# twke18/SPML

Measured on AMD Instinct MI355X. Metric: images/sec (513x513) + k-means iters/sec, higher is better.
Workload: dtype f32

## Files before the change

### include/spml_hip.h

```cpp
#ifndef SPML_HIP_H_
#define SPML_HIP_H_

#include <stddef.h>
#include <stdint.h>

#ifdef __cplusplus
extern "C" {
#endif

typedef enum spml_status {
  SPML_OK = 0,
  SPML_ERR_INVALID_ARG = -1,
  SPML_ERR_UNSUPPORTED = -2,
  SPML_ERR_WORKSPACE = -3,
  SPML_ERR_LAUNCH = -4
} spml_status;

const char* spml_status_string(int status);

#define SPML_ABI_VERSION 8
int spml_abi_version(void);

int spml_set_deterministic(int on);
int spml_get_deterministic(void);
// ... 337 lines not shown

int spml_bn_bwd_hl8_f32(const float* dy, const float* y, const unsigned char* relu_mask,
                        const float* x, int64_t R, int C, const float* mean,
                        const float* invstd, const float* gamma, const float* cmax,
                        const float* cmin, float* d_gamma, float* d_beta, float* dx,
                        void* dx_hl8, float* dx_bound, float* d_residual, void* ws,
                        size_t ws_bytes, void* stream);

int spml_bn_bwd_hl8_chunks_f32(const float* dy, const unsigned char* relu_mask, const float* x,
                               const float* chunk_stats, int chunks, int chunk_rows, int64_t R,
                               int C, const float* mean, const float* invstd, const float* gamma,
                               const float* cmax, const float* cmin, float* d_gamma,
                               float* d_beta, float* max_dz, float* dx, void* dx_hl8,
                               float* dx_bound, float* d_residual, void* stream);

int spml_bn_act_bwd_reduce_ext_chunks_f32(const float* chunk_stats, int chunks, int chunk_rows,
                                          int64_t R, int C, const float* invstd, float* sum_dz,
                                          float* sum_dz_xhat, float* max_dz, void* stream);

int spml_conv_hl8_pyramid_f32(const void* a, const float* a_bound, const void* b,
                              const float* b_bound, const float* bias, const float* addend,
                              float* out,
                              int n_img, int H, int W, int K, int N, int groups,
                              const int* dilations, void* stream);
int spml_hl8_weight_transposed_into_f32(const float* w, int Cout, int taps, int Cin,
                                        const float* bound, void* out, int taps_total,
                                        int tap_offset, void* stream);
int spml_absmax_bound_f32(const float* x, int64_t n, float* bound, int zero_first,
                          void* stream);

int spml_hl8_weight_set_f32(const float* const* w, const int* cout, const int* cin,
                            const int* taps, int n, float* bounds, void* const* fwd,
                            void* const* transposed, void* stream);

int spml_bn_finalize_ranks_f32(const float* stats, int world, int C, float eps,
                               float momentum, float* running_mean, float* running_var,
                               float* mean, float* invstd, float* total_count, void* stream);

int spml_conv_hl8_affine_f32(const void* a, const float* a_bound, const void* b,
                             const float* b_bound, const float* bias, const float* addend,
                             int relu, float* out, float* out_bound, int n_img, int H,
                             int W, int K, int N, int taps, int dilation, void* stream);

int spml_upsample_ce_supported(int C);
size_t spml_upsample_ce_workspace_bytes(int N, int H, int W);
int spml_upsample_ce_fwd_f32(const float* logits, const int64_t* labels, int N, int C, int h,
                             int w, int H, int W, int64_t ignore_index, float* lse,
                             float* result, void* ws, size_t ws_bytes, void* stream);
int spml_upsample_ce_bwd_f32(const float* logits, const int64_t* labels, const float* lse,
                             int N, int C, int h, int w, int H, int W, int64_t ignore_index,
                             const float* scale, float* d_logits, void* stream);
const char* spml_upsample_ce_bwd_path_name(int N, int C, int h, int w, int H, int W);


int spml_unit_hl8_from_nchw_f32(const float* x, int n, int C, int h, int w, void* out,
                                void* stream);

int spml_class_head_supported(int Ch, int ncls);

int spml_class_head_accumulate_f32(const float* hidden, int Ch, int h, int w,
                                   const float* weight, const float* bias, int ncls,
                                   float* canvas, int Hp, int Wp, int sh, int sw,
                                   void* stream);

int spml_argmax_channels_i64(const float* canvas, int ncls, int Hp, int Wp, int h, int w,
                             int64_t* out, void* stream);
// ... 103 lines not shown
```

### spml_amd/_ffi.py

```python
import ctypes
import os
import threading
from ctypes import c_char_p, c_double, c_float, c_int, c_int64, c_size_t, c_void_p

import torch

_HERE = os.path.dirname(os.path.abspath(__file__))
LIB_PATH = os.environ.get('SPML_HIP_LIB') or os.path.join(_HERE, 'lib', 'libspml_hip.so')

_lib = None
_lock = threading.Lock()

_P = c_void_p
_SIGNATURES = {
    'spml_status_string': (c_char_p, [c_int]),
    'spml_abi_version': (c_int, []),
    'spml_normalize_concat_loc_f32': (c_int, [_P, c_int, c_int, c_int, c_int, _P, _P, _P, _P, _P]),
    'spml_normalize_concat_loc_bwd_f32': (c_int, [_P, c_int, c_int, c_int, c_int, _P, _P, _P, _P, _P, _P]),
    'spml_normalize_concat_local_f32': (c_int, [_P, c_int, c_int, c_int, c_int, _P, c_int, _P, _P, _P, _P]),
    'spml_normalize_concat_local_nhwc_supported': (c_int, [c_int, c_int]),
    'spml_normalize_concat_local_nhwc_f32': (c_int, [_P, c_int, c_int, c_int, c_int, _P, c_int, _P, _P, _P, _P]),
    'spml_normalize_concat_local_nhwc_bwd_f32': (c_int, [_P, c_int, c_int, c_int, c_int, _P, c_int, _P, _P, _P,
                                                         _P, _P]),
    'spml_normalize_concat_local_bwd_f32': (c_int, [_P, c_int, c_int, c_int, c_int, _P, c_int, _P, _P, _P,
# ... 59 lines not shown
                                                   c_int, c_int, c_int, _P, _P, _P]),
    'spml_bn_bwd_hl8_chunks_f32': (c_int, [_P, _P, _P, _P, c_int, c_int, c_int64, c_int, _P, _P, _P, _P, _P, _P, _P, _P,
                                           _P, _P, _P, _P, _P]),
    'spml_bn_act_bwd_reduce_ext_chunks_f32': (c_int, [_P, c_int, c_int, c_int64, c_int, _P, _P, _P, _P, _P]),
    'spml_conv_wgrad_hl8_supported': (c_int, [c_int, c_int, c_int]),
    'spml_conv_wgrad_workspace_bytes': (c_size_t, [c_int, c_int, c_int, c_int, c_int, c_int]),
    'spml_conv_wgrad_hl8_f32': (c_int, [_P, _P, _P, _P, _P, c_int, c_int, c_int, c_int, c_int, c_int, c_int, _P,
                                        c_size_t, _P]),
    'spml_conv_wgrad_pyramid_hl8_supported': (c_int, [c_int, c_int, c_int]),
    'spml_conv_tap_gather_f32': (c_int, [_P, _P, _P, c_int, c_int, c_int, c_int, c_int, _P, _P]),
    'spml_conv_wgrad_pyramid_workspace_bytes': (c_size_t, [c_int, c_int, c_int, c_int, c_int, c_int]),
    'spml_conv_wgrad_pyramid_hl8_f32': (c_int, [_P, _P, _P, _P, _P, c_int, c_int, c_int, c_int, c_int, c_int, _P, _P,
                                                c_size_t, _P]),
    'spml_conv_hl8_path_name': (c_char_p, [c_int, c_int, c_int, c_int, c_int, c_int, c_int, c_int]),
    'spml_conv_wgrad_path_name': (c_char_p, [c_int, c_int, c_int, c_int, c_int, c_int, c_int]),
    'spml_conv_wgrad_splits': (c_int, [c_int, c_int, c_int, c_int, c_int, c_int, c_int]),
    'spml_bn_stats_ext_f32': (c_int, [_P, c_int64, c_int, _P, _P, _P, _P, _P, c_size_t, _P]),
    'spml_bn_stats_ext_chunks_f32': (c_int, [_P, c_int, c_int, c_int64, c_int, _P, _P, _P, _P, _P]),
    'spml_bn_finalize_f32': (c_int, [_P, _P, c_int, c_double, c_float, c_float, _P, _P, _P, _P]),
    'spml_bn_act_apply_hl8_f32': (c_int, [_P, _P, _P, c_int64, c_int, _P, _P, _P, _P, _P, _P, c_int, _P, _P, _P, _P,
                                          _P]),
    'spml_bn_act_bwd_reduce_ext_f32': (c_int, [_P, _P, _P, _P, c_int64, c_int, _P, _P, _P, _P, _P, _P, c_size_t, _P]),
    'spml_bn_act_bwd_apply_hl8_f32': (c_int, [_P, _P, _P, _P, c_int64, c_int, _P, _P, _P, _P, _P, _P, _P, _P,
                                              c_double, _P, _P, _P, _P, _P, _P]),
    'spml_bn_fwd_hl8_f32': (c_int, [_P, _P, _P, c_int64, c_int, _P, _P, _P, _P, c_float, c_float, c_int, _P, _P, _P, _P,
                                    _P, _P, _P, _P, _P, c_size_t, _P]),
    'spml_bn_bwd_hl8_f32': (c_int, [_P, _P, _P, _P, c_int64, c_int, _P, _P, _P, _P, _P, _P, _P, _P, _P, _P, _P, _P,
                                    c_size_t, _P]),
    'spml_conv_hl8_pyramid_f32': (c_int, [_P, _P, _P, _P, _P, _P, _P, c_int, c_int, c_int, c_int, c_int, c_int, _P,
                                          _P]),
    'spml_hl8_weight_transposed_into_f32': (c_int, [_P, c_int, c_int, c_int, _P, _P, c_int, c_int, _P]),
    'spml_absmax_bound_f32': (c_int, [_P, c_int64, _P, c_int, _P]),
    'spml_hl8_weight_set_f32': (c_int, [_P, _P, _P, _P, c_int, _P, _P, _P, _P]),
    'spml_bn_finalize_ranks_f32': (c_int, [_P, c_int, c_int, c_float, c_float, _P, _P, _P, _P, _P, _P]),
    'spml_conv_hl8_affine_f32': (c_int, [_P, _P, _P, _P, _P, _P, c_int, _P, _P, c_int, c_int, c_int, c_int, c_int,
                                         c_int, c_int, _P]),
    'spml_upsample_ce_supported': (c_int, [c_int]),
    'spml_upsample_ce_workspace_bytes': (c_size_t, [c_int, c_int, c_int]),
    'spml_upsample_ce_fwd_f32': (c_int, [_P, _P, c_int, c_int, c_int, c_int, c_int, c_int, c_int64, _P, _P, _P,
                                         c_size_t, _P]),
    'spml_upsample_ce_bwd_f32': (c_int, [_P, _P, _P, c_int, c_int, c_int, c_int, c_int, c_int, c_int64, _P, _P, _P]),
    'spml_upsample_ce_bwd_path_name': (c_char_p, [c_int, c_int, c_int, c_int, c_int, c_int]),
    'spml_bn_stats_f32': (c_int, [_P, c_int64, c_int, _P, _P, _P, c_size_t, _P]),
    'spml_bn_act_apply_f32': (c_int, [_P, _P, c_int64, c_int, _P, _P, _P, _P, c_int, _P, _P]),
    'spml_bn_act_bwd_reduce_f32': (c_int, [_P, _P, _P, c_int64, c_int, _P, _P, _P, _P, _P, c_size_t, _P]),
    'spml_bn_act_bwd_apply_f32': (c_int, [_P, _P, _P, c_int64, c_int, _P, _P, _P, _P, _P, c_double, _P, _P, _P,
                                          _P]),
    'spml_clock_probe': (c_int, [_P, c_int, _P]),
    'spml_maxpool3x3s2_nhwc_f32': (c_int, [_P, c_int, c_int, c_int, c_int, _P, _P]),
    'spml_window_accumulate_f32': (c_int, [_P, c_int, c_int, c_int, _P, _P, c_int, c_int, c_int, c_int,
                                           _P]),
    'spml_unit_hl8_from_nchw_f32': (c_int, [_P, c_int, c_int, c_int, c_int, _P, _P]),
    'spml_class_head_supported': (c_int, [c_int, c_int]),
    'spml_class_head_accumulate_f32': (c_int, [_P, c_int, c_int, c_int, _P, _P, c_int, _P, c_int, c_int, c_int, c_int,
                                               _P]),
    'spml_argmax_channels_i64': (c_int, [_P, c_int, c_int, c_int, c_int, c_int, _P, _P]),
    'spml_iou_counts_i64': (c_int, [_P, _P, c_int64, c_int, _P, _P]),
    'spml_resample_unit_f32': (c_int, [_P, c_int, c_int, c_int, c_int64, c_int64, c_int64, c_int, c_int, c_int, c_int,
                                       c_int, _P, c_int, c_int, _P]),
    'spml_resample_classes_accumulate_f32': (c_int, [_P, c_int, c_int, c_int, c_int64, c_int64, c_int64, c_int, c_int,
                                                     c_int, c_int, c_int, c_int, _P, _P]),
    'spml_cam_finalize_f32': (c_int, [_P, c_int, c_int64, c_int, c_int, _P, c_int, c_float, _P, _P]),
    'spml_upsample_argmax_i64': (c_int, [_P, c_int, c_int, c_int, c_int, c_int, _P, _P]),
    'spml_view_probs_accumulate_f32': (c_int, [_P, c_int, c_int, c_int, _P, _P, c_int, c_int, c_int, c_int, c_int, _P,
                                               _P]),
    'spml_view_votes_workspace_bytes': (c_size_t, [c_int, c_int]),
# ... 1152 lines not shown
                                  versions=tuple(wt._version for wt in weights), operand=operand)
  z = conv_hl8(x, operand, n_img, h, w, 1)
  bias = None
  if any(bb is not None for bb in biases):
    bias = sum(bb.detach() for bb in biases if bb is not None).contiguous()
  out = torch.empty((n_img, cout, h, w), dtype=torch.float32, device=dev, memory_format=torch.channels_last)
  dil = (ctypes.c_int * groups)(*[int(d) for d in dilations])
  check(lib().spml_conv_tap_gather_f32(_ptr_any(z), _dp(bias), _ptr_any(out), n_img, h, w, cout, groups,
                                       ctypes.cast(dil, c_void_p), stream_ptr()), 'spml_conv_tap_gather_f32')
  return out


def hl8_weight_set(weights):
  import ctypes
  n = len(weights)
  dev = weights[0].device
  wl = [wt.detach().contiguous(memory_format=torch.channels_last) for wt in weights]
  bounds = torch.empty((4,), dtype=torch.float32, device=dev)
  shapes = [(wt.shape[0], wt.shape[1], wt.shape[2] * wt.shape[3]) for wt in wl]
  fwd = [torch.empty((co * ci * t * 4,), dtype=torch.uint8, device=dev) for co, ci, t in shapes]
  tr = [torch.empty((co * ci * t * 4,), dtype=torch.uint8, device=dev) for co, ci, t in shapes]
  pv, iv = ctypes.c_void_p * n, ctypes.c_int * n
  check(lib().spml_hl8_weight_set_f32(
      pv(*[wt.data_ptr() for wt in wl]), iv(*[sh[0] for sh in shapes]), iv(*[sh[1] for sh in shapes]),
      iv(*[sh[2] for sh in shapes]), n, _dp(bounds), pv(*[t.data_ptr() for t in fwd]),
      pv(*[t.data_ptr() for t in tr]), stream_ptr()), 'spml_hl8_weight_set_f32')
  out = []
  for i, (co, ci, t) in enumerate(shapes):
    b = bounds[i:i + 1]
    out.append((Hl8(fwd[i], b, co, t * ci), Hl8(tr[i], b, ci, t * co)))
  return out


def conv_hl8_affine(a, b, bias, n_img, h, w, taps, dilation=1, addend=None, relu=True, want_hl8=True):
  k, n = a.channels, b.rows
  if a.rows != n_img * h * w or b.channels != taps * k:
    raise SpmlHipError('conv_hl8_affine: operand shapes do not match')
  dev = a.data.device
  out = torch.empty((n_img, n, h, w), dtype=torch.float32, device=dev, memory_format=torch.channels_last)
  bound = _f32(1, dev) if want_hl8 else None
  check(lib().spml_conv_hl8_affine_f32(ptr(a.data), _dp(a.bound), ptr(b.data), _dp(b.bound), ptr(bias, torch.float32),
                                       _ptr_any(addend, True), int(bool(relu)), _ptr_any(out), _dp(bound), n_img, h, w,
                                       k, n, taps, dilation, stream_ptr()), 'spml_conv_hl8_affine_f32')
  return out, (hl8_from_f32(out, bound=bound) if want_hl8 else None)


def upsample_ce_supported(c):
  return bool(lib().spml_upsample_ce_supported(int(c)))


def upsample_ce_bwd_path_name(n, c, h, w, hh, ww):
  return lib().spml_upsample_ce_bwd_path_name(int(n), int(c), int(h), int(w), int(hh), int(ww)).decode()


def upsample_ce_fwd(logits_nhwc, labels, ignore_index):
  n, h, w, c = logits_nhwc.shape
  hh, ww = labels.shape[-2:]
  lse = torch.empty((n, hh, ww), dtype=torch.float32, device=logits_nhwc.device)
  result = torch.empty((3,), dtype=torch.float32, device=logits_nhwc.device)
  ws = workspace(lib().spml_upsample_ce_workspace_bytes(n, hh, ww), logits_nhwc.device)
  check(lib().spml_upsample_ce_fwd_f32(ptr(logits_nhwc, torch.float32), ptr(labels, torch.int64), n, c, h, w, hh, ww,
                                       int(ignore_index), ptr(lse), ptr(result), ptr(ws), ws.numel(), stream_ptr()),
        'spml_upsample_ce_fwd_f32')
  return result, lse


# ... 281 lines not shown
```

### spml_amd/csrc/conv.hip

```cpp
#include "common.hpp"

#include <math.h>
#include <stdlib.h>

#ifndef SPML_CONV_EXP
#define SPML_CONV_EXP 0
#endif

namespace spml {
namespace {

constexpr int BSTAT_BATCH = 8;

typedef const __attribute__((address_space(1))) void* gptr_t;
typedef __attribute__((address_space(3))) void* lptr_t;

__device__ uint4 g_zero_page[16];

__device__ __forceinline__ float pow2_scale(float bound) {
  if (!(bound > 0.f) || bound > 1e38f) return 1.f;
  int e;
  (void)frexpf(bound, &e);
  e = 14 - e;
  e = e < -100 ? -100 : (e > 100 ? 100 : e);
// ... 90 lines not shown
  for (int o = 32; o > 0; o >>= 1) m = fmaxf(m, __shfl_xor(m, o, kWave));
  if ((threadIdx.x & 63) == 0) sm[threadIdx.x >> 6] = m;
  __syncthreads();
  if (threadIdx.x == 0)
    atomicMax(reinterpret_cast<unsigned*>(ws.bound + wi), __float_as_uint(fmaxf(fmaxf(sm[0], sm[1]), fmaxf(sm[2], sm[3]))));
}

__global__ __launch_bounds__(256) void weightset_convert(const WeightSet ws) {
  const int64_t total = ws.start[ws.n];
  for (int64_t i = (int64_t)blockIdx.x * 256 + threadIdx.x; i < total; i += (int64_t)gridDim.x * 256) {
    int wi = 0;
    while (wi + 1 < ws.n && i >= ws.start[wi + 1]) ++wi;
    const int64_t u = i - ws.start[wi];
    const int cout = ws.cout[wi], cin = ws.cin[wi], taps = ws.taps[wi];
    const float s = pow2_scale(ws.bound[wi]);
    const float4v v0 = reinterpret_cast<const float4v*>(ws.w[wi])[2 * u];
    const float4v v1 = reinterpret_cast<const float4v*>(ws.w[wi])[2 * u + 1];
    const float v[8] = {v0[0], v0[1], v0[2], v0[3], v1[0], v1[1], v1[2], v1[3]};
    union { half8 h; uint4 q; _Float16 e[8]; } hh, ll;
    split_unscaled(v, s, hh.h, ll.h);
    ws.fwd[wi][2 * u] = hh.q;
    ws.fwd[wi][2 * u + 1] = ll.q;
    const int c8 = cin >> 3;
    const int ci0 = (int)(u % c8) * 8;
    const int64_t rest = u / c8;
    const int tap = (int)(rest % taps), co = (int)(rest / taps);
    const int tapo = taps - 1 - tap;
    _Float16* th = reinterpret_cast<_Float16*>(ws.tr[wi]);
#pragma unroll
    for (int e = 0; e < 8; ++e) {
      const size_t tu = ((size_t)(ci0 + e) * taps + tapo) * (cout >> 3) + (co >> 3);
      th[(2 * tu) * 8 + (co & 7)] = hh.e[e];
      th[(2 * tu + 1) * 8 + (co & 7)] = ll.e[e];
    }
  }
}

struct ConvArgs {
  const uint4* a;
  const uint4* b;
  const float* a_bound;
  const float* b_bound;
  const float* addend;
  const unsigned char* addend_mask;
  const float* bias;
  int relu;
  float* out_bound;
  float* out;
  int64_t R;
  int H, W, K, N, taps, dil;
  int n_col_tiles, n_tiles;
  int dils[4];
  int tap_groups;
  float* stats;
  float* stats_zero;
  const float* bstat_x;
  const unsigned char* bstat_mask;
  const float* bstat_mean;
  float* bstats;
};

template <int RB, int kStages, int WGS, int RG, bool CHUNK = false, int NC = 4, bool BSTAT = false, bool BADD = false>
__global__ __launch_bounds__(64 * NC * RG, WGS) void conv_gemm(const ConvArgs a) {
  static_assert(!BSTAT || (RG == 1 && NC == 4), "backward statistics: a wave owns its 64 columns over the whole tile");
  static_assert(!BADD || (BSTAT && !CHUNK), "the addend form exists for the un-chunked backward statistics only");
  constexpr int kABlocks = 2 * RB * RG;
// ... 874 lines not shown
  hipLaunchKernelGGL(hl8_convert_wt, dim3(grid), dim3(256), 0, (hipStream_t)stream, w, Cout, taps, Cin, bound,
                     static_cast<uint4*>(out), taps_total, tap_offset);
  return launch_status();
}

extern "C" int spml_hl8_weight_set_f32(const float* const* w, const int* cout, const int* cin, const int* taps,
                                       int n, float* bounds, void* const* fwd, void* const* transposed,
                                       void* stream) {
  if (!w || !cout || !cin || !taps || !bounds || !fwd || !transposed || n < 1 || n > 4) return SPML_ERR_INVALID_ARG;
  WeightSet ws{};
  ws.n = n;
  ws.bound = bounds;
  int64_t acc = 0, largest = 0;
  for (int i = 0; i < n; ++i) {
    if (!w[i] || !fwd[i] || !transposed[i] || cout[i] <= 0 || cin[i] <= 0 || (taps[i] != 1 && taps[i] != 9))
      return SPML_ERR_INVALID_ARG;
    if ((cout[i] & 7) || (cin[i] & 7) || !al16(w[i]) || !al16(fwd[i]) || !al16(transposed[i])) return SPML_ERR_UNSUPPORTED;
    ws.w[i] = w[i];
    ws.fwd[i] = static_cast<uint4*>(fwd[i]);
    ws.tr[i] = static_cast<uint4*>(transposed[i]);
    ws.cout[i] = cout[i]; ws.cin[i] = cin[i]; ws.taps[i] = taps[i];
    ws.start[i] = acc;
    const int64_t units = (int64_t)cout[i] * cin[i] * taps[i] / 8;
    acc += units;
    largest = std::max(largest, units);
  }
  for (int i = n; i <= 4; ++i) ws.start[i] = acc;
  hipStream_t s = (hipStream_t)stream;
  if (hipMemsetAsync(bounds, 0, 4 * sizeof(float), s) != hipSuccess) return SPML_ERR_LAUNCH;
  const int gx = (int)std::min<int64_t>(256, (largest * 2 + 255) / 256);
  hipLaunchKernelGGL(weightset_absmax, dim3(gx, n), dim3(256), 0, s, ws);
  const int grid = (int)std::min<int64_t>(4096, (acc + 255) / 256);
  hipLaunchKernelGGL(weightset_convert, dim3(grid), dim3(256), 0, s, ws);
  return launch_status();
}

extern "C" int spml_absmax_bound_f32(const float* x, int64_t n, float* bound, int zero_first, void* stream) {
  if (!x || !bound || n <= 0) return SPML_ERR_INVALID_ARG;
  if (!al16(x)) return SPML_ERR_UNSUPPORTED;
  hipStream_t s = (hipStream_t)stream;
  if (zero_first && hipMemsetAsync(bound, 0, sizeof(float), s) != hipSuccess) return SPML_ERR_LAUNCH;
  const int grid = (int)std::min<int64_t>(2048, (n / 4 + 255) / 256 + 1);
  hipLaunchKernelGGL(absmax_bound, dim3(grid), dim3(256), 0, s, x, n, reinterpret_cast<unsigned*>(bound));
  return launch_status();
}

extern "C" int spml_conv_hl8_supported(int K, int N, int taps) {
  return (taps == 1 || taps == 9) && K > 0 && (K & 15) == 0 && N > 0 && (N & 63) == 0;
}

extern "C" int spml_conv_hl8_f32(const void* a, const float* a_bound, const void* b, const float* b_bound,
                                 const float* addend, const unsigned char* addend_mask, float* out, int n_img,
                                 int H, int W, int K, int N, int taps, int dilation, void* stream) {
  if (!a || !b || !out || n_img <= 0 || H <= 0 || W <= 0 || dilation < 1) return SPML_ERR_INVALID_ARG;
  if (!spml_conv_hl8_supported(K, N, taps) || !al16(a) || !al16(b) || !al16(out) || (addend && !al16(addend)))
    return SPML_ERR_UNSUPPORTED;
  ConvArgs c{};
  c.a = static_cast<const uint4*>(a);
  c.b = static_cast<const uint4*>(b);
  c.a_bound = a_bound;
  c.b_bound = b_bound;
  c.addend = addend;
  c.addend_mask = addend ? addend_mask : nullptr;
  c.out = out;
  c.R = (int64_t)n_img * H * W;
  c.H = H; c.W = W; c.K = K; c.N = N; c.taps = taps; c.dil = dilation;
// ... 320 lines not shown
```

### spml_amd/mc_bottleneck.py

```python
import os

import torch
import torch.distributed as dist

from spml_amd import _ffi
from spml_amd._cache import BoundedCache


def _group_of(bn):
  if isinstance(bn, torch.nn.SyncBatchNorm) and dist.is_available() and dist.is_initialized():
    return bn.process_group if bn.process_group is not None else dist.group.WORLD
  return None


def available(block, x, allow_forward_only=True):
  if os.environ.get('SPML_NO_MC_CONV') == '1' or not (x.is_cuda and x.dtype == torch.float32 and x.dim() == 4):
    return False
  if not block.training or block.stride != 1 or not x.is_contiguous(memory_format=torch.channels_last):
    return False
  convs = [block.conv1, block.conv2, block.conv3] + ([block.downsample[0]] if block.downsample is not None else [])
  if os.environ.get('SPML_MC_NARROW_UNITS') == '0' and any(
      (c.in_channels & 255) or (c.out_channels & 255) for c in convs):
    return False
  bns = [block.bn1, block.bn2, block.bn3] + ([block.downsample[1]] if block.downsample is not None else [])
# ... 176 lines not shown
  side.wait_stream(main)
  with torch.cuda.stream(side):
    dw = _ffi.conv_wgrad_hl8(dy, x, n, h, w, taps, dil)
  dy.data.record_stream(side)
  dy.bound.record_stream(side)
  dw.record_stream(main)
  return dw


def handover_mode():
  return 0 if os.environ.get('SPML_BN3_HANDOVER') == '0' else 1


class _Handover(object):
  taken = 0

  def __init__(self):
    self.bn3 = None
    self.dx = self.stats = self.version = None

  def put(self, dx, stats):
    self.dx, self.stats, self.version = dx, stats, dx._version

  def take(self, d_out):
    dx, stats, version = self.dx, self.stats, self.version
    self.dx = self.stats = self.version = None
    if dx is None or d_out._version != version or d_out.data_ptr() != dx.data_ptr() or d_out.shape != dx.shape or \
        d_out.stride() != dx.stride() or d_out.dtype != dx.dtype:
      return None
    _Handover.taken += 1
    return stats


class _Unit(torch.autograd.Function):

  @staticmethod
  def forward(ctx, block, x, xh_data, xh_bound, w1, g1, b1, w2, g2, b2, w3, g3, b3, wd, gd, bd, hand_out=None,
              hand_in=None, *p_bn3):
    n, cin, h, w = x.shape
    rows = n * h * w
    dil = block.conv2.dilation[0]
    width, cout = w1.shape[0], w3.shape[0]
    xh = _ffi.Hl8(xh_data, xh_bound, rows, cin) if xh_data is not None else _ffi.hl8_from_f32(x)
    wset = _ffi.hl8_weight_set([w1, w2, w3] + ([wd] if wd is not None else []))
    (w1f, w1t), (w2f, w2t), (w3f, w3t) = wset[:3]
    conv = _ffi.conv_hl8_stats
    a1, s1 = conv(xh, w1f, n, h, w, 1)
    counters = []
    n1 = _Bn(block.bn1, a1, rows, width, chunk_stats=s1, counters=counters)
    a2, s2 = conv(n1.yh, w2f, n, h, w, 9, dil)
    n2 = _Bn(block.bn2, a2, rows, width, chunk_stats=s2, counters=counters)
    a3, s3 = conv(n2.yh, w3f, n, h, w, 1)
    nd = ad = wdt = None
    ex3 = None
    if wd is not None:
      wdf, wdt = wset[3]
      ad, sd = conv(xh, wdf, n, h, w, 1)
      ex3, exd = sync_pair(block.bn3, a3, s3, block.downsample[1], ad, sd, rows, cout)
      nd = _Bn(block.downsample[1], ad, rows, cout, relu=False, want_f32=True, want_hl8=False, chunk_stats=sd,
               counters=counters, gathered=exd)
      residual, res_bound = nd.y, nd.bound
    else:
      residual, res_bound = x, xh.bound
    n3 = _Bn(block.bn3, a3, rows, cout, residual=residual, residual_bound=res_bound, want_f32=True, chunk_stats=s3,
             counters=counters, gathered=ex3)
    bump_counters(counters)
    ctx.block, ctx.geom = block, (n, cin, h, w, dil, width, cout)
    ctx.bn_meta = [(m.count, m.group, m.world) for m in (n1, n2, n3)] + \
        ([(nd.count, nd.group, nd.world)] if nd is not None else [])
    tensors = [xh.data, xh.bound, a1, n1.yh.data, n1.yh.bound, a2, n2.yh.data, n2.yh.bound, a3, n3.mask,
               n1.mask, n2.mask,
               w1t.data, w1t.bound, w2t.data, w2t.bound, w3t.data, w3t.bound, g1, g2, g3]
    tensors += list(n1.saved) + list(n2.saved) + list(n3.saved)
    if nd is not None:
      tensors += [ad, wdt.data, wdt.bound, gd] + list(nd.saved)
    ctx.hand_in = ctx.hand_out = None
    if hand_in is not None and len(p_bn3) == 3 and p_bn3[0] is not None and n3.world == 1 and \
# ... 54 lines not shown
    dw1 = _wgrad(side, da1, xh, n, h, w, 1)
    dx = None
    if p_bn3 is not None and need_x and handover_mode():
      last = lambda dy, wt, **kw: _ffi.conv_hl8_bwd_stats(dy, wt, n, h, w, 1, 1, p_bn3[0], p_bn3[1], p_bn3[2], **kw)
    else:
      last = lambda dy, wt, **kw: (_ffi.conv_hl8(dy, wt, n, h, w, 1, **kw), None)
    cx = None
    if has_ds:
      ad, wdt_d, wdt_b, gd = t[33:37]
      sd = t[37:41]
      if not pair:
        _, dad, _, dgd, dbd = _bn_backward(dres, ad, rows, cout, gd, sd, m[3][0], m[3][1], m[3][2], None)
      dwd = _wgrad(side, dad, xh, n, h, w, 1)
      if need_x:
        dx = _ffi.conv_hl8(da1, w1t, n, h, w, 1)
        dx, cx = last(dad, H(wdt_d, wdt_b, cin, cout), addend=dx)
    elif need_x:
      dx, cx = last(da1, w1t, addend=d_out, addend_mask=m3)
    if cx is not None:
      ctx.hand_in.put(dx, cx)
    if side is not None:
      torch.cuda.current_stream().wait_stream(side)
    return (None, dx, None, None, dw1, dg1, db1, dw2, dg2, db2, dw3, dg3, db3, dwd, dgd, dbd) + (None,) * 5


class _ConvBnAct(torch.autograd.Function):

  @staticmethod
  def forward(ctx, conv, bn, x, weight, gamma, beta):
    n, cin, h, w = x.shape
    rows, cout = n * h * w, weight.shape[0]
    taps, dil = weight.shape[2] * weight.shape[3], conv.dilation[0]
    xh = getattr(x, '_spml_hl8', None) or _ffi.hl8_from_f32(x)
    (wf, wt), = _ffi.hl8_weight_set([weight])
    a, st = _ffi.conv_hl8_stats(xh, wf, n, h, w, taps, dil)
    nb = _Bn(bn, a, rows, cout, relu=True, want_f32=True, want_hl8=False, chunk_stats=st)
    ctx.geom = (n, cin, h, w, taps, dil, cout)
    ctx.bn_meta = (nb.count, nb.group, nb.world)
    ctx.save_for_backward(xh.data, xh.bound, a, nb.mask, wt.data, wt.bound, gamma, *nb.saved)
    return nb.y

  @staticmethod
  def backward(ctx, dy):
    n, cin, h, w, taps, dil, cout = ctx.geom
    rows = n * h * w
    xh_d, xh_b, a, mask, wt_d, wt_b, gamma = ctx.saved_tensors[:7]
    saved = ctx.saved_tensors[7:11]
    if not dy.is_contiguous(memory_format=torch.channels_last):
      dy = dy.contiguous(memory_format=torch.channels_last)
    count, group, world = ctx.bn_meta
    _, da, _, dg, db = _bn_backward(dy, a, rows, cout, gamma, saved, count, group, world, mask)
    side = _side_stream(dy.device)
    dw = _wgrad(side, da, _ffi.Hl8(xh_d, xh_b, rows, cin), n, h, w, taps, dil)
    dx = None
    if ctx.needs_input_grad[2]:
      dx = _ffi.conv_hl8(da, _ffi.Hl8(wt_d, wt_b, cin, taps * cout), n, h, w, taps, dil)
    if side is not None:
      torch.cuda.current_stream().wait_stream(side)
    return None, None, dx, dw, dg, db


def conv_bn_act_available(conv, bn, x):
  if os.environ.get('SPML_NO_MC_CONV') == '1' or not (x.is_cuda and x.dtype == torch.float32 and x.dim() == 4):
    return False
  if not (bn.training and torch.is_grad_enabled() and x.is_contiguous(memory_format=torch.channels_last)):
    return False
  k = conv.kernel_size
# ... 29 lines not shown
```

### spml_amd/nn/optimizer.py

```python
import torch
from torch.optim.optimizer import Optimizer, required


class SGD(Optimizer):

  def __init__(self, params, lr=required, momentum=0, dampening=0, weight_decay=0,
               nesterov=False):
    if nesterov and (momentum <= 0 or dampening != 0):
      raise ValueError('Nesterov momentum requires a momentum and zero dampening')
    assert dampening == 0, 'not implemented'
    defaults = dict(lr=lr, momentum=momentum, dampening=dampening,
                    weight_decay=weight_decay, nesterov=nesterov)
    super().__init__(params, defaults)

  @torch.no_grad()
  def step(self, lr, closure=None):
    loss = None
    if closure is not None:
      with torch.enable_grad():
        loss = closure()
    for group in self.param_groups:
      params = [p for p in group['params'] if p.grad is not None]
      if not params:
        continue
      grads = [p.grad for p in params]
      wd, mom, scale = group['weight_decay'], group['momentum'], group['lr'] * lr
      if wd != 0:
        grads = torch._foreach_add(grads, params, alpha=wd)
      if mom != 0:
        bufs = []
        for p in params:
          st = self.state[p]
          if 'momentum_buffer' not in st:
            st['momentum_buffer'] = torch.zeros_like(p)
          bufs.append(st['momentum_buffer'])
        torch._foreach_mul_(bufs, mom)
        torch._foreach_add_(bufs, grads, alpha=scale)
        if group['nesterov']:
          upd = torch._foreach_add(grads, bufs, alpha=mom)
        else:
          upd = bufs
        torch._foreach_sub_(params, upd)
      else:
        torch._foreach_sub_(params, grads)
    return loss
```

### spml_amd/train.py

```python
import os

import torch
import torch.distributed as dist

import spml_amd.models.utils as model_utils
import spml_amd.utils.general.train as train_utils
from spml_amd import parallel
from spml_amd.models.embeddings.resnet_deeplab import resnet_50_deeplab, resnet_101_deeplab
from spml_amd.models.embeddings.resnet_pspnet import resnet_50_pspnet, resnet_101_pspnet
from spml_amd.models.predictions import segsort as segsort_plain
from spml_amd.models.predictions import segsort_softmax
from spml_amd.nn.optimizer import SGD

LOSS_KEYS = ('sem_ann_loss', 'sem_occ_loss', 'img_sim_loss', 'feat_aff_loss')


def build_models(config, softmax_head=True, recipe='voc'):
  backbone = config.network.backbone_types
  if recipe == 'densepose':
    import spml_amd.models.embeddings.resnet_pspnet_densepose as dp_emb
    import spml_amd.models.predictions.segsort_softmax_densepose as dp_pred
    makers = {'panoptic_pspnet_101': dp_emb.resnet_101_pspnet,
              'panoptic_pspnet_50': dp_emb.resnet_50_pspnet}
    if backbone not in makers:
# ... 12 lines not shown
  else:
    raise ValueError('Not support ' + str(backbone))
  if config.network.prediction_types == 'segsort':
    prediction_model = (segsort_softmax if softmax_head else segsort_plain).segsort(config)
  else:
    raise ValueError('Not support ' + str(config.network.prediction_types))
  return embedding_model, prediction_model


class Trainer:

  def __init__(self, config, device, softmax_head=True, freeze_unused=True,
               channels_last=False, recipe='voc', models=None):
    self.config = config
    self.device = torch.device(device)
    self.distributed = parallel.is_distributed()
    self.world = dist.get_world_size() if self.distributed else 1
    emb, pred = models if models is not None else build_models(config, softmax_head, recipe)
    if freeze_unused:
      for name in ('conv1', 'res2'):
        for p in getattr(emb.resnet_backbone, name).parameters():
          p.requires_grad_(False)
    emb, pred = emb.to(self.device), pred.to(self.device)
    if channels_last:
      emb = emb.to(memory_format=torch.channels_last)
      pred = pred.to(memory_format=torch.channels_last)
    if config.network.use_syncbn and self.distributed:
      emb = torch.nn.SyncBatchNorm.convert_sync_batchnorm(emb)
      pred = torch.nn.SyncBatchNorm.convert_sync_batchnorm(pred)
    self.embedding_model, self.prediction_model = emb, pred
    self.optimizer = SGD(emb.get_params_lr() + pred.get_params_lr(), lr=1,
                         momentum=config.train.momentum,
                         weight_decay=config.train.weight_decay)
    self.emb_fwd, self.pred_fwd = emb, pred
    if self.distributed:
      ids = [self.device.index] if self.device.type == 'cuda' else None
      ddp = dict(device_ids=ids, broadcast_buffers=not config.network.use_syncbn,
                 gradient_as_bucket_view=True, bucket_cap_mb=64)
      self.emb_fwd = torch.nn.parallel.DistributedDataParallel(emb, **ddp)
      if any(p.requires_grad for p in pred.parameters()):
        self.pred_fwd = torch.nn.parallel.DistributedDataParallel(pred, **ddp)
    self.memory_banks = {}
    self.curr_iter = config.train.begin_iteration
    if self.device.type == 'cuda':
      from spml_amd import _ffi
      if _ffi.deterministic():
        from spml_amd.nn.conv import make_deterministic
        make_deterministic(self.embedding_model)
        make_deterministic(self.prediction_model)
      if _ffi.deterministic() and os.environ.get('SPML_DETERMINISTIC_FRAMEWORK') == '1':
        torch.backends.cudnn.deterministic = True
        torch.backends.cudnn.benchmark = False

  def lr(self, it):
    t = self.config.train
    if t.lr_policy == 'step':
      return train_utils.lr_step(t.base_lr, it, t.decay_iterations, t.warmup_iteration)
    return train_utils.lr_poly(t.base_lr, it, t.max_iteration, t.warmup_iteration)

  def forward_losses(self, datas, targets):
    targets = dict(targets)
    emb = self.emb_fwd(datas, targets)
    protos = model_utils.local_prototypes(
        emb['cluster_embedding'], emb['cluster_embedding_with_loc'], emb['cluster_index'],
        emb['cluster_batch_index'], emb['cluster_semantic_label'], emb['cluster_instance_label'])
    (targets['prototype'], targets['prototype_with_loc'], targets['prototype_semantic_label'],
# ... 52 lines not shown
        'prediction_model': self.prediction_model.state_dict(),
        'optimizer': self.optimizer.state_dict(),
        'memory_banks': self.memory_banks,
        'iteration': self.curr_iter,
    }



class ClassifierTrainer:

  def __init__(self, config, device, channels_last=False, models=None):
    from spml_amd.models.predictions.softmax_classifier import softmax_classifier
    self.config = config
    self.device = torch.device(device)
    self.distributed = parallel.is_distributed()
    if models is not None:
      emb, pred = models
    else:
      if config.network.prediction_types != 'softmax_classifier':
        raise ValueError('Not support ' + str(config.network.prediction_types))
      makers = {'panoptic_pspnet_101': resnet_101_pspnet, 'panoptic_deeplab_101': resnet_101_deeplab}
      if config.network.backbone_types not in makers:
        raise ValueError('Not support ' + str(config.network.backbone_types))
      emb, pred = makers[config.network.backbone_types](config), softmax_classifier(config)
    emb, pred = emb.to(self.device), pred.to(self.device)
    if channels_last:
      emb = emb.to(memory_format=torch.channels_last)
      pred = pred.to(memory_format=torch.channels_last)
    if config.network.use_syncbn and self.distributed:
      pred = torch.nn.SyncBatchNorm.convert_sync_batchnorm(pred)
    self.embedding_model, self.prediction_model = emb, pred
    self.optimizer = SGD(emb.get_params_lr() + pred.get_params_lr(), lr=1,
                         momentum=config.train.momentum, weight_decay=config.train.weight_decay)
    if self.device.type == 'cuda':
      from spml_amd import _ffi
      if _ffi.deterministic():
        from spml_amd.nn.conv import make_deterministic
        make_deterministic(pred)
        make_deterministic(emb)
    self.pred_fwd = pred
    if self.distributed:
      ids = [self.device.index] if self.device.type == 'cuda' else None
      self.pred_fwd = torch.nn.parallel.DistributedDataParallel(
          pred, device_ids=ids, broadcast_buffers=not config.network.use_syncbn)
    self.curr_iter = config.train.begin_iteration

  lr = Trainer.lr

  def load_pretrained(self, path_or_state):
    state = path_or_state
    if isinstance(state, (str, bytes)) or hasattr(state, '__fspath__'):
      state = torch.load(state, map_location=self.device, weights_only=True)
    if 'embedding_model' not in state:
      raise ValueError('Pre-trained model is required.')
    self.embedding_model.load_state_dict(state['embedding_model'], resume=True)

  def step(self, datas, targets):
    self.embedding_model.eval()
    self.prediction_model.train()
    with torch.no_grad():
      embeddings = self.embedding_model.generate_embeddings(datas, targets)
    outputs = self.pred_fwd({'embedding': embeddings['embedding']}, targets)
    loss = outputs['sem_ann_loss']
    lr = self.lr(self.curr_iter)
    self.optimizer.zero_grad()
    loss.backward()
# ... 66 lines not shown
```

Before: 147.6.

## Batch per-step weight splitting into one table launch and fuse SGD updates

Adds a multi-tensor SGD kernel that updates every parameter, with weight decay and momentum, in a few launches instead of per-tensor PyTorch ops. It also adds a forward pre-hook that, at the start of each model forward, converts all conv weights seen in the previous forward to the split half format in one batched absmax/convert pass. Convolution units then look those results up instead of launching per-block conversions. The aim is to cut kernel launch and Python overhead. The cost is extra hook bookkeeping, and the weight table only takes effect after the first forward has recorded which weights were requested.

```diff
diff --git a/include/spml_hip.h b/include/spml_hip.h
--- a/include/spml_hip.h
+++ b/include/spml_hip.h
@@ -393,6 +393,14 @@
 int spml_hl8_weight_set_f32(const float* const* w, const int* cout, const int* cin,
                             const int* taps, int n, float* bounds, void* const* fwd,
                             void* const* transposed, void* stream);
+
+int spml_hl8_weight_table_f32(const float* const* w, const int* cout, const int* cin,
+                              const int* taps, int n, float* bounds, void* const* fwd,
+                              void* const* transposed, void* stream);
+
+int spml_sgd_step_f32(void* const* p, const void* const* grad, void* const* buf,
+                      const int64_t* numel, const float* scale, const float* weight_decay,
+                      const float* momentum, int n, void* stream);
 
 int spml_bn_finalize_ranks_f32(const float* stats, int world, int C, float eps,
                                float momentum, float* running_mean, float* running_var,
diff --git a/spml_amd/_ffi.py b/spml_amd/_ffi.py
--- a/spml_amd/_ffi.py
+++ b/spml_amd/_ffi.py
@@ -115,6 +115,8 @@
     'spml_hl8_weight_transposed_into_f32': (c_int, [_P, c_int, c_int, c_int, _P, _P, c_int, c_int, _P]),
     'spml_absmax_bound_f32': (c_int, [_P, c_int64, _P, c_int, _P]),
     'spml_hl8_weight_set_f32': (c_int, [_P, _P, _P, _P, c_int, _P, _P, _P, _P]),
+    'spml_hl8_weight_table_f32': (c_int, [_P, _P, _P, _P, c_int, _P, _P, _P, _P]),
+    'spml_sgd_step_f32': (c_int, [_P, _P, _P, _P, _P, _P, _P, c_int, _P]),
     'spml_bn_finalize_ranks_f32': (c_int, [_P, c_int, c_int, c_float, c_float, _P, _P, _P, _P, _P, _P]),
     'spml_conv_hl8_affine_f32': (c_int, [_P, _P, _P, _P, _P, _P, c_int, _P, _P, c_int, c_int, c_int, c_int, c_int,
                                          c_int, c_int, _P]),
@@ -1333,6 +1335,44 @@
   return out
 
 
+def hl8_weight_table(weights):
+  import ctypes
+  n = len(weights)
+  dev = weights[0].device
+  wl = [wt.detach().contiguous(memory_format=torch.channels_last) for wt in weights]
+  shapes = [(wt.shape[0], wt.shape[1], wt.shape[2] * wt.shape[3]) for wt in wl]
+  sizes = [co * ci * t * 4 for co, ci, t in shapes]
+  offs = [0]
+  for sz in sizes:
+    offs.append(offs[-1] + (sz + 255) // 256 * 256)
+  bounds = torch.empty((n,), dtype=torch.float32, device=dev)
+  fwd = torch.empty((offs[-1],), dtype=torch.uint8, device=dev)
+  tr = torch.empty((offs[-1],), dtype=torch.uint8, device=dev)
+  pv, iv = ctypes.c_void_p * n, ctypes.c_int * n
+  f0, t0 = fwd.data_ptr(), tr.data_ptr()
+  check(lib().spml_hl8_weight_table_f32(
+      pv(*[wt.data_ptr() for wt in wl]), iv(*[sh[0] for sh in shapes]), iv(*[sh[1] for sh in shapes]),
+      iv(*[sh[2] for sh in shapes]), n, _dp(bounds), pv(*[f0 + o for o in offs[:-1]]),
+      pv(*[t0 + o for o in offs[:-1]]), stream_ptr()), 'spml_hl8_weight_table_f32')
+  out = []
+  for i, (co, ci, t) in enumerate(shapes):
+    b = bounds[i:i + 1]
+    out.append((Hl8(fwd[offs[i]:offs[i] + sizes[i]], b, co, t * ci), Hl8(tr[offs[i]:offs[i] + sizes[i]], b, ci, t * co)))
+  return out
+
+
+def sgd_step(params, grads, bufs, scales, weight_decays, momenta):
+  import ctypes
+  n = len(params)
+  if n == 0:
+    return
+  pv, fv = ctypes.c_void_p * n, ctypes.c_float * n
+  check(lib().spml_sgd_step_f32(
+      pv(*[t.data_ptr() for t in params]), pv(*[t.data_ptr() for t in grads]),
+      pv(*[None if t is None else t.data_ptr() for t in bufs]), (ctypes.c_int64 * n)(*[t.numel() for t in params]),
+      fv(*scales), fv(*weight_decays), fv(*momenta), n, stream_ptr()), 'spml_sgd_step_f32')
+
+
 def conv_hl8_affine(a, b, bias, n_img, h, w, taps, dilation=1, addend=None, relu=True, want_hl8=True):
   k, n = a.channels, b.rows
   if a.rows != n_img * h * w or b.channels != taps * k:
diff --git a/spml_amd/csrc/conv.hip b/spml_amd/csrc/conv.hip
--- a/spml_amd/csrc/conv.hip
+++ b/spml_amd/csrc/conv.hip
@@ -146,6 +146,101 @@
       const size_t tu = ((size_t)(ci0 + e) * taps + tapo) * (cout >> 3) + (co >> 3);
       th[(2 * tu) * 8 + (co & 7)] = hh.e[e];
       th[(2 * tu + 1) * 8 + (co & 7)] = ll.e[e];
+    }
+  }
+}
+
+struct WeightRow {
+  const float* w;
+  uint4* fwd;
+  uint4* tr;
+  float* bound;
+  int32_t cout, cin, taps;
+};
+constexpr int WT_ROWS = 72;
+struct WeightBatch {
+  WeightRow row[WT_ROWS];
+  int start[WT_ROWS + 1];
+  int n;
+};
+static_assert(sizeof(WeightBatch) <= 4000, "the batch must fit the kernel argument segment");
+
+constexpr int WT_CO = 64, WT_CI = 32;
+constexpr int WT_LD = WT_CO + 8;
+
+__device__ __forceinline__ int weighttable_row(const WeightBatch& b) {
+  int wi = 0, hi = b.n;
+  while (hi - wi > 1) {
+    const int mid = (wi + hi) >> 1;
+    if ((int)blockIdx.x >= b.start[mid]) wi = mid; else hi = mid;
+  }
+  return wi;
+}
+
+__global__ __launch_bounds__(256) void weighttable_absmax(const WeightBatch b) {
+  __shared__ float sm[4];
+  const int wi = weighttable_row(b);
+  const WeightRow& r = b.row[wi];
+  const int q = (int)blockIdx.x - b.start[wi];
+  const int cout = r.cout, cin = r.cin, taps = r.taps;
+  const int ci_tiles = (cin + WT_CI - 1) / WT_CI;
+  const int ci0 = (q % ci_tiles) * WT_CI;
+  const int tap = (q / ci_tiles) % taps, co0 = (q / ci_tiles / taps) * WT_CO;
+  const int co = co0 + (threadIdx.x >> 2), ci = ci0 + (threadIdx.x & 3) * 8;
+  float m = 0.f;
+  if (co < cout && ci < cin) {
+    const int64_t u = (((int64_t)co * taps + tap) * cin + ci) >> 3;
+    const float4v v0 = reinterpret_cast<const float4v*>(r.w)[2 * u];
+    const float4v v1 = reinterpret_cast<const float4v*>(r.w)[2 * u + 1];
+    m = fmaxf(fmaxf(fmaxf(fabsf(v0[0]), fabsf(v0[1])), fmaxf(fabsf(v0[2]), fabsf(v0[3]))),
+              fmaxf(fmaxf(fabsf(v1[0]), fabsf(v1[1])), fmaxf(fabsf(v1[2]), fabsf(v1[3]))));
+  }
+#pragma unroll
+  for (int o = 32; o > 0; o >>= 1) m = fmaxf(m, __shfl_xor(m, o, kWave));
+  if ((threadIdx.x & 63) == 0) sm[threadIdx.x >> 6] = m;
+  __syncthreads();
+  if (threadIdx.x == 0)
+    atomicMax(reinterpret_cast<unsigned*>(r.bound), __float_as_uint(fmaxf(fmaxf(sm[0], sm[1]), fmaxf(sm[2], sm[3]))));
+}
+
+__global__ __launch_bounds__(256) void weighttable_convert(const WeightBatch b) {
+  __shared__ __attribute__((aligned(16))) _Float16 lh[WT_CI * WT_LD];
+  __shared__ __attribute__((aligned(16))) _Float16 ll[WT_CI * WT_LD];
+  const int wi = weighttable_row(b);
+  const WeightRow& r = b.row[wi];
+  const int q = (int)blockIdx.x - b.start[wi];
+  const int cout = r.cout, cin = r.cin, taps = r.taps;
+  const int ci_tiles = (cin + WT_CI - 1) / WT_CI;
+  const int ci0 = (q % ci_tiles) * WT_CI;
+  const int tap = (q / ci_tiles) % taps, co0 = (q / ci_tiles / taps) * WT_CO;
+  const float s = pow2_scale(*r.bound);
+  {
+    const int co = co0 + (threadIdx.x >> 2), ci = ci0 + (threadIdx.x & 3) * 8;
+    if (co < cout && ci < cin) {
+      const int64_t u = (((int64_t)co * taps + tap) * cin + ci) >> 3;
+      const float4v v0 = reinterpret_cast<const float4v*>(r.w)[2 * u];
+      const float4v v1 = reinterpret_cast<const float4v*>(r.w)[2 * u + 1];
+      const float v[8] = {v0[0], v0[1], v0[2], v0[3], v1[0], v1[1], v1[2], v1[3]};
+      union { half8 h; uint4 q; _Float16 e[8]; } hh, lo;
+      split_unscaled(v, s, hh.h, lo.h);
+      r.fwd[2 * u] = hh.q;
+      r.fwd[2 * u + 1] = lo.q;
+#pragma unroll
+      for (int e = 0; e < 8; ++e) {
+        lh[((threadIdx.x & 3) * 8 + e) * WT_LD + (threadIdx.x >> 2)] = hh.e[e];
+        ll[((threadIdx.x & 3) * 8 + e) * WT_LD + (threadIdx.x >> 2)] = lo.e[e];
+      }
+    }
+  }
+  __syncthreads();
+  {
+    const int cil = threadIdx.x >> 3, cb = threadIdx.x & 7;
+    const int ci = ci0 + cil, co = co0 + cb * 8;
+    if (ci < cin && co < cout) {
+      const int tapo = taps - 1 - tap;
+      const int64_t tu = ((int64_t)ci * taps + tapo) * (cout >> 3) + (co >> 3);
+      r.tr[2 * tu] = *reinterpret_cast<const uint4*>(&lh[cil * WT_LD + cb * 8]);
+      r.tr[2 * tu + 1] = *reinterpret_cast<const uint4*>(&ll[cil * WT_LD + cb * 8]);
     }
   }
 }
@@ -1086,6 +1181,45 @@
   hipLaunchKernelGGL(weightset_absmax, dim3(gx, n), dim3(256), 0, s, ws);
   const int grid = (int)std::min<int64_t>(4096, (acc + 255) / 256);
   hipLaunchKernelGGL(weightset_convert, dim3(grid), dim3(256), 0, s, ws);
+  return launch_status();
+}
+
+extern "C" int spml_hl8_weight_table_f32(const float* const* w, const int* cout, const int* cin, const int* taps,
+                                         int n, float* bounds, void* const* fwd, void* const* transposed,
+                                         void* stream) {
+  if (!w || !cout || !cin || !taps || !bounds || !fwd || !transposed || n < 1) return SPML_ERR_INVALID_ARG;
+  for (int i = 0; i < n; ++i) {
+    if (!w[i] || !fwd[i] || !transposed[i] || cout[i] <= 0 || cin[i] <= 0 || (taps[i] != 1 && taps[i] != 9))
+      return SPML_ERR_INVALID_ARG;
+    if ((cout[i] & 7) || (cin[i] & 7) || !al16(w[i]) || !al16(fwd[i]) || !al16(transposed[i])) return SPML_ERR_UNSUPPORTED;
+    if ((int64_t)((cout[i] + WT_CO - 1) / WT_CO) * ((cin[i] + WT_CI - 1) / WT_CI) * taps[i] > (1 << 24))
+      return SPML_ERR_UNSUPPORTED;
+  }
+  hipStream_t s = (hipStream_t)stream;
+  if (hipMemsetAsync(bounds, 0, (size_t)n * sizeof(float), s) != hipSuccess) return SPML_ERR_LAUNCH;
+  WeightBatch b;
+  b.n = 0;
+  b.start[0] = 0;
+  auto flush = [&]() {
+    if (b.n > 0) {
+      hipLaunchKernelGGL(weighttable_absmax, dim3(b.start[b.n]), dim3(256), 0, s, b);
+      hipLaunchKernelGGL(weighttable_convert, dim3(b.start[b.n]), dim3(256), 0, s, b);
+    }
+    b.n = 0;
+  };
+  for (int i = 0; i < n; ++i) {
+    const int tiles = ((cout[i] + WT_CO - 1) / WT_CO) * ((cin[i] + WT_CI - 1) / WT_CI) * taps[i];
+    if (b.n == WT_ROWS || b.start[b.n] + (int64_t)tiles > (1 << 26)) flush();
+    WeightRow& r = b.row[b.n];
+    r.w = w[i];
+    r.fwd = static_cast<uint4*>(fwd[i]);
+    r.tr = static_cast<uint4*>(transposed[i]);
+    r.bound = bounds + i;
+    r.cout = cout[i]; r.cin = cin[i]; r.taps = taps[i];
+    b.start[b.n + 1] = b.start[b.n] + tiles;
+    ++b.n;
+  }
+  flush();
   return launch_status();
 }
 
diff --git a/spml_amd/csrc/sgd.hip b/spml_amd/csrc/sgd.hip
--- /dev/null
+++ b/spml_amd/csrc/sgd.hip
@@ -0,0 +1,117 @@
+#include "common.hpp"
+
+#include <algorithm>
+
+namespace spml {
+namespace {
+
+constexpr int SGD_TENSORS = 60;
+constexpr int SGD_CHUNK = 8192;
+
+struct SgdBatch {
+  float* p[SGD_TENSORS];
+  const float* g[SGD_TENSORS];
+  float* buf[SGD_TENSORS];
+  int64_t n[SGD_TENSORS];
+  float scale[SGD_TENSORS], wd[SGD_TENSORS], mom[SGD_TENSORS];
+  int first[SGD_TENSORS + 1];
+  int count;
+};
+static_assert(sizeof(SgdBatch) <= 4000, "the batch must fit the kernel argument segment");
+
+struct SgdScalars {
+  float scale, wd, mom;
+  bool has_wd, has_mom;
+};
+
+__device__ __forceinline__ void sgd_one(float& p, float g, float& buf, const SgdScalars& s) {
+#pragma clang fp contract(off)
+  if (s.has_wd) g = __builtin_fmaf(s.wd, p, g);
+  if (s.has_mom) {
+    buf = buf * s.mom;
+    buf = __builtin_fmaf(s.scale, g, buf);
+    p = p - buf;
+  } else {
+    p = p - g;
+  }
+}
+
+__global__ __launch_bounds__(256) void sgd_step(const SgdBatch b) {
+  int t = 0, hi = b.count;
+  while (hi - t > 1) {
+    const int mid = (t + hi) >> 1;
+    if ((int)blockIdx.x >= b.first[mid]) t = mid; else hi = mid;
+  }
+  const int64_t off = (int64_t)((int)blockIdx.x - b.first[t]) * SGD_CHUNK;
+  const int len = (int)std::min<int64_t>(SGD_CHUNK, b.n[t] - off);
+  float* __restrict__ p = b.p[t] + off;
+  const float* __restrict__ g = b.g[t] + off;
+  float* __restrict__ buf = b.buf[t] ? b.buf[t] + off : nullptr;
+  SgdScalars s;
+  s.scale = b.scale[t]; s.wd = b.wd[t]; s.mom = b.mom[t];
+  s.has_wd = s.wd != 0.f;
+  s.has_mom = buf != nullptr;
+  const bool vec = (((uintptr_t)p | (uintptr_t)g | (uintptr_t)buf) & 15) == 0;
+  const int n4 = vec ? len >> 2 : 0;
+  for (int i = threadIdx.x; i < n4; i += 256) {
+    float4v pv = reinterpret_cast<const float4v*>(p)[i];
+    const float4v gv = reinterpret_cast<const float4v*>(g)[i];
+    float4v bv = {0.f, 0.f, 0.f, 0.f};
+    if (s.has_mom) bv = reinterpret_cast<const float4v*>(buf)[i];
+#pragma unroll
+    for (int e = 0; e < 4; ++e) {
+      float pe = pv[e], be = bv[e];
+      sgd_one(pe, gv[e], be, s);
+      pv[e] = pe; bv[e] = be;
+    }
+    reinterpret_cast<float4v*>(p)[i] = pv;
+    if (s.has_mom) reinterpret_cast<float4v*>(buf)[i] = bv;
+  }
+  for (int i = (n4 << 2) + threadIdx.x; i < len; i += 256) {
+    float pe = p[i], be = s.has_mom ? buf[i] : 0.f;
+    sgd_one(pe, g[i], be, s);
+    p[i] = pe;
+    if (s.has_mom) buf[i] = be;
+  }
+}
+
+}
+}
+
+using namespace spml;
+
+extern "C" int spml_sgd_step_f32(void* const* p, const void* const* grad, void* const* buf, const int64_t* numel,
+                                 const float* scale, const float* weight_decay, const float* momentum, int n,
+                                 void* stream) {
+  if (n < 0) return SPML_ERR_INVALID_ARG;
+  if (n > 0 && (!p || !grad || !buf || !numel || !scale || !weight_decay || !momentum)) return SPML_ERR_INVALID_ARG;
+  for (int i = 0; i < n; ++i) {
+    if (!p[i] || !grad[i] || numel[i] < 0) return SPML_ERR_INVALID_ARG;
+    if ((momentum[i] != 0.f) != (buf[i] != nullptr)) return SPML_ERR_INVALID_ARG;
+    if (!(momentum[i] >= 0.f)) return SPML_ERR_UNSUPPORTED;
+    if (((uintptr_t)p[i] | (uintptr_t)grad[i] | (uintptr_t)buf[i]) & 3) return SPML_ERR_INVALID_ARG;
+    if ((numel[i] + SGD_CHUNK - 1) / SGD_CHUNK > (1 << 24)) return SPML_ERR_UNSUPPORTED;
+  }
+  hipStream_t s = (hipStream_t)stream;
+  SgdBatch b;
+  b.count = 0;
+  b.first[0] = 0;
+  auto flush = [&]() {
+    if (b.count > 0) hipLaunchKernelGGL(sgd_step, dim3(b.first[b.count]), dim3(256), 0, s, b);
+    b.count = 0;
+  };
+  for (int i = 0; i < n; ++i) {
+    if (numel[i] == 0) continue;
+    const int blocks = (int)((numel[i] + SGD_CHUNK - 1) / SGD_CHUNK);
+    if (b.count == SGD_TENSORS || b.first[b.count] + (int64_t)blocks > (1 << 26)) flush();
+    const int k = b.count++;
+    b.p[k] = static_cast<float*>(p[i]);
+    b.g[k] = static_cast<const float*>(grad[i]);
+    b.buf[k] = static_cast<float*>(buf[i]);
+    b.n[k] = numel[i];
+    b.scale[k] = scale[i]; b.wd[k] = weight_decay[i]; b.mom[k] = momentum[i];
+    b.first[k + 1] = b.first[k] + blocks;
+  }
+  flush();
+  return launch_status();
+}
diff --git a/spml_amd/mc_bottleneck.py b/spml_amd/mc_bottleneck.py
--- a/spml_amd/mc_bottleneck.py
+++ b/spml_amd/mc_bottleneck.py
@@ -232,6 +232,11 @@
     return stats
 
 
+def _weight_set(conv, weights):
+  split = getattr(conv, '_spml_split', None)
+  return (split.lookup(weights) if split is not None else None) or _ffi.hl8_weight_set(weights)
+
+
 class _Unit(torch.autograd.Function):
 
   @staticmethod
@@ -242,7 +247,7 @@
     dil = block.conv2.dilation[0]
     width, cout = w1.shape[0], w3.shape[0]
     xh = _ffi.Hl8(xh_data, xh_bound, rows, cin) if xh_data is not None else _ffi.hl8_from_f32(x)
-    wset = _ffi.hl8_weight_set([w1, w2, w3] + ([wd] if wd is not None else []))
+    wset = _weight_set(block.conv1, [w1, w2, w3] + ([wd] if wd is not None else []))
     (w1f, w1t), (w2f, w2t), (w3f, w3t) = wset[:3]
     conv = _ffi.conv_hl8_stats
     a1, s1 = conv(xh, w1f, n, h, w, 1)
@@ -363,7 +368,7 @@
     rows, cout = n * h * w, weight.shape[0]
     taps, dil = weight.shape[2] * weight.shape[3], conv.dilation[0]
     xh = getattr(x, '_spml_hl8', None) or _ffi.hl8_from_f32(x)
-    (wf, wt), = _ffi.hl8_weight_set([weight])
+    (wf, wt), = _weight_set(conv, [weight])
     a, st = _ffi.conv_hl8_stats(xh, wf, n, h, w, taps, dil)
     nb = _Bn(bn, a, rows, cout, relu=True, want_f32=True, want_hl8=False, chunk_stats=st)
     ctx.geom = (n, cin, h, w, taps, dil, cout)
diff --git a/spml_amd/nn/optimizer.py b/spml_amd/nn/optimizer.py
--- a/spml_amd/nn/optimizer.py
+++ b/spml_amd/nn/optimizer.py
@@ -1,5 +1,74 @@
+import os
+
 import torch
 from torch.optim.optimizer import Optimizer, required
+
+
+def fused_enabled():
+  return os.environ.get('SPML_FUSED_SGD') != '0'
+
+
+def _dense(t):
+  return t.is_contiguous() or (t.dim() == 4 and t.is_contiguous(memory_format=torch.channels_last))
+
+
+def _order(t):
+  return tuple(st for sz, st in zip(t.shape, t.stride()) if sz != 1)
+
+
+class _Root(object):
+
+  def __init__(self):
+    self.asked = {}
+    self.ready = {}
+
+  def __deepcopy__(self, memo):
+    return _Root()
+
+  def __reduce__(self):
+    return (_Root, ())
+
+  def begin(self, module, args):
+    weights, self.asked, self.ready = list(self.asked.values()), {}, {}
+    if not weights or not fused_enabled():
+      return
+    dev = weights[0].device
+    if not all(w.is_cuda and w.device == dev and w.dtype == torch.float32 and w.dim() == 4 for w in weights):
+      return
+    from spml_amd import _ffi
+    with torch.cuda.device(dev):
+      ops = _ffi.hl8_weight_table(weights)
+    self.ready = {id(w): (w, w.data_ptr(), w._version, op) for w, op in zip(weights, ops)}
+
+  def end(self, module, args, output):
+    self.ready = {}
+
+  def lookup(self, weights):
+    for w in weights:
+      self.asked[id(w)] = w
+    out = []
+    for w in weights:
+      hit = self.ready.get(id(w))
+      if hit is None or hit[0] is not w or hit[1] != w.data_ptr() or hit[2] != w._version:
+        return None
+      out.append(hit[3])
+    return out
+
+
+class SplitWeightCache(object):
+
+  def __init__(self):
+    self.roots = []
+
+  def attach(self, model):
+    root = _Root()
+    model.register_forward_pre_hook(root.begin)
+    model.register_forward_hook(root.end, always_call=True)
+    for m in model.modules():
+      if isinstance(m, torch.nn.Conv2d):
+        m._spml_split = root
+    self.roots.append(root)
+    return root
 
 
 class SGD(Optimizer):
@@ -12,6 +81,40 @@
     defaults = dict(lr=lr, momentum=momentum, dampening=dampening,
                     weight_decay=weight_decay, nesterov=nesterov)
     super().__init__(params, defaults)
+    self.split_cache = SplitWeightCache()
+
+  def __setstate__(self, state):
+    super().__setstate__(state)
+    self.__dict__.setdefault('split_cache', SplitWeightCache())
+
+  def _fused_plan(self, lr):
+    if not fused_enabled():
+      return None
+    ps, gs, bufs, scales, wds, moms = [], [], [], [], [], []
+    for group in self.param_groups:
+      wd, mom, scale = group['weight_decay'], group['momentum'], group['lr'] * lr
+      if group['nesterov'] or mom < 0:
+        return None
+      for p in group['params']:
+        g = p.grad
+        if g is None:
+          continue
+        if not (p.is_cuda and g.is_cuda and p.dtype == torch.float32 and g.dtype == torch.float32 and
+                g.layout == torch.strided and p.device == g.device and p.device.index == torch.cuda.current_device() and
+                _dense(p) and g.shape == p.shape and _order(g) == _order(p)):
+          return None
+        buf = None
+        if mom != 0:
+          st = self.state[p]
+          buf = st.get('momentum_buffer')
+          if buf is None:
+            buf = st['momentum_buffer'] = torch.zeros_like(p)
+          if not (buf.is_cuda and buf.dtype == torch.float32 and buf.device == p.device and buf.shape == p.shape and
+                  _order(buf) == _order(p)):
+            return None
+        ps.append(p); gs.append(g); bufs.append(buf)
+        scales.append(scale); wds.append(wd); moms.append(mom)
+    return ps, gs, bufs, scales, wds, moms
 
   @torch.no_grad()
   def step(self, lr, closure=None):
@@ -19,6 +122,14 @@
     if closure is not None:
       with torch.enable_grad():
         loss = closure()
+    plan = self._fused_plan(lr)
+    if plan is not None:
+      from spml_amd import _ffi
+      _ffi.sgd_step(*plan)
+      touched = plan[0] + [b for b in plan[2] if b is not None]
+      if touched:
+        torch.autograd.graph.increment_version(touched)
+      return loss
     for group in self.param_groups:
       params = [p for p in group['params'] if p.grad is not None]
       if not params:
diff --git a/spml_amd/train.py b/spml_amd/train.py
--- a/spml_amd/train.py
+++ b/spml_amd/train.py
@@ -68,6 +68,8 @@
     self.optimizer = SGD(emb.get_params_lr() + pred.get_params_lr(), lr=1,
                          momentum=config.train.momentum,
                          weight_decay=config.train.weight_decay)
+    for model in (emb, pred):
+      self.optimizer.split_cache.attach(model)
     self.emb_fwd, self.pred_fwd = emb, pred
     if self.distributed:
       ids = [self.device.index] if self.device.type == 'cuda' else None
@@ -186,6 +188,8 @@
     self.embedding_model, self.prediction_model = emb, pred
     self.optimizer = SGD(emb.get_params_lr() + pred.get_params_lr(), lr=1,
                          momentum=config.train.momentum, weight_decay=config.train.weight_decay)
+    for model in (emb, pred):
+      self.optimizer.split_cache.attach(model)
     if self.device.type == 'cuda':
       from spml_amd import _ffi
       if _ffi.deterministic():
```

Result: no change. 149.0, median of 6 (+1.0%).
